# aehogan/lammps-induced-dipole-polarization-pair-style

Measured on AMD Instinct MI355X. Metric: atom-steps/sec, higher is better.
Workload: dtype f64

## Files before the change

lammps-induced-dipole-polarization-pair-style_amd/csrc/lab/api_env_knobs.inc:

```
  if (const char *e = getenv("POLAR_ABLATE")) h->ablate = atoi(e);
  if (const char *e = getenv("POLAR_HOST_COLORS")) h->host_colors = atoi(e) != 0;
  if (const char *e = getenv("POLAR_SWEEP_KERNEL")) h->sweep_kernel = atoi(e);
  if (const char *e = getenv("POLAR_TILE_WAVES")) h->tile_waves = atoi(e) == 8 ? 8 : 4;
  if (const char *e = getenv("POLAR_TILE_WIDE")) h->tile_wide = atoi(e) != 0;
  if (const char *e = getenv("POLAR_CACHE_R2")) h->cache_r2 = atoi(e);
  if (const char *e = getenv("POLAR_LJ_TYPED")) h->lj_typed = atoi(e) != 0;
  if (const char *e = getenv("POLAR_STATIC_XQ")) h->static_xq = atoi(e) != 0;
  if (const char *e = getenv("POLAR_POL_FIRST")) h->pol_first = atoi(e) != 0;
  if (const char *e = getenv("POLAR_LP_WG_PER_CU")) h->lp_wg_per_cu = atoi(e);
  if (const char *e = getenv("POLAR_LP_QM")) h->lp_quad_major = atoi(e) != 0;
  if (const char *e = getenv("POLAR_LP_TILES")) h->lp_tiles = atoi(e) == 1 ? 1 : 2;
  if (const char *e = getenv("POLAR_LP_ROWS")) h->lp_rows = std::max(1, std::min(64, atoi(e)));
  if (const char *e = getenv("POLAR_LP_PAIRS")) h->lp_pairs = atoi(e) != 0;
  if (const char *e = getenv("POLAR_CLUSTER_DIST")) h->cluster_dist = atof(e);
  if (const char *e = getenv("POLAR_CLUSTER_MAX")) h->cluster_max = std::max(1, std::min(4, atoi(e)));
  if (const char *e = getenv("POLAR_LP_DEPTH")) { int v = atoi(e); h->lp_depth = (v == 2 || v == 3) ? v : 0; }
  if (const char *e = getenv("POLAR_QUAD_BLOCK")) { int v = atoi(e); if (v >= 64 && v <= 1024 && v % 64 == 0) h->quad_block = v; }
  if (const char *e = getenv("POLAR_FIELD_BLOCK")) { int v = atoi(e); if (v >= 64 && v <= 1024 && v % 64 == 0) h->field_block = v; }
  if (const char *e = getenv("POLAR_FORCE_LITERAL")) h->force_literal = atoi(e) != 0;
```

lammps-induced-dipole-polarization-pair-style_amd/csrc/polar_handle.hpp:

```cpp
#pragma once
#include <hip/hip_runtime.h>

#include <algorithm>
#include <initializer_list>
#include <utility>
#include <chrono>
#include <cmath>
#include <cstdio>
#include <cstdlib>
#include <exception>
#include <cstring>
#include <numeric>
#include <string>
#include <thread>
#include <mutex>
#include <condition_variable>
#include <functional>
#include <memory>
#include <stdexcept>
#include <unistd.h>
#include <vector>

#include "pair_host.hpp"
#include "polar_kernels.hpp"
// ... 117 lines not shown
  DBuf<double2> d_dd_s;
  DBuf<int2> d_lpdesc;
  DBuf<double> d_lp_pend;
  DBuf<double> d_lp_part;
  int lp_npart = 0;
  DBuf<int> d_slot;
  std::vector<int> h_cl;
  DBuf<int> d_cl_orig, d_cl_cnt, d_cl_wrap, d_cl_tw;
  DBuf<int4> d_cl_s;
  long long cl_pitch = 0;
  int ncl = 0;
  double cluster_dist = 2.0;
  int cluster_max = 4;
  long long cl_slots = 0;
  DBuf<double4> d_xq, d_pos4, d_xq_s;
  long long nl_pairs = 0, dd_pairs = 0;
  long long nl_pitch = 0, dd_pitch = 0;
  DBuf<int> d_overflow;
  DBuf<unsigned long long> d_ddtot;
  int *h_flags = nullptr;
  unsigned long long *h_ddtot = nullptr;
  int inum = 0;
  long long nneigh = 0;
  bool mu_resident = false;
  DBuf<double> d_dbgf;
  DBuf<double> d_acc_x, d_acc_f, d_acc_g, d_acc_dF, d_acc_dG, d_acc_part;
  DBuf<AccelState> d_acc_state;
  long long acc_pitch = 0; int acc_rows = 0;
  DBuf<double> d_mu0;
  bool mu0_saved = false;
  int attempt = 0;
  int last_sweeps = 0;
  bool mu_host_in_sync = false;
  std::vector<int> color_off;
  std::vector<int> color_sub;
  int color_nsub = 1;
  DBuf<int> d_bflag; int bflag_n = 0;
  std::vector<int *> h_nl_stage; std::vector<hipEvent_t> ev_nl;
  hipStream_t up_stream = nullptr; hipEvent_t ev_list_up = nullptr; bool list_up_pending = false;
  std::vector<long long> h_first; std::vector<int> h_nn, h_ilist;
  bool colors_global = false;
  std::vector<int> user_colors;
  bool user_colors_clashed = false;
  std::vector<int> h_rows;
  bool colors_valid = false;
  double color_keep = 2.0;
  bool slots_by_color = false;
  long long color_epoch = 0;
  long long slots_epoch = -1;
  bool colors_recheck = false;
  std::vector<int> h_color;
  DBuf<int> d_color_orig, d_color_s;
  DBuf<int> d_klist;
  DBuf<int> d_cadj, d_cdeg, d_ccnt, d_cflags, d_crelabel;
  DBuf<unsigned long long> d_cprio;
  DBuf<double> d_cstat;
  DBuf<long long> d_coff;
  int *h_cflags = nullptr;
  double *h_cstat = nullptr;
  long long *h_coff = nullptr;
  int cadj_pitch = 16;
  int host_colors = 0;
  int colors_reused = 0, colors_rebuilt = 0;
  double ms_color_host = 0.0;
  double color_dist = 2.4;
  int field_block = 256;
  double bbox_lo[3] = {0, 0, 0}, bbox_hi[3] = {0, 0, 0};
  long long global_count = 0;
  DBuf<double> d_xchg; DBuf<int> d_xidx;
  bool device_list = false;
  int user_full_list = 0;
  long long lj_pitch = 0;
  DBuf<double4> d_ljpos; DBuf<int2> d_ljaux; DBuf<int> d_tag, d_nspecial, d_special, d_ljcell_id, d_ljcell_cnt, d_ljcell_fill; DBuf<long long> d_ljcell_first; DBuf<double> d_cutneighsq;
  int lj_typed = 1;
  bool lj_tab_arith = false;
  int lj_pers = 1;
  int ncu = 0;
  int lj_pers_threads = 768;
  bool sym_typed = false, dev_typed = false;
  int static_xq = 1;
  int pol_first = 1;
#ifdef POLAR_LAB
  int force_literal = 0;
#endif
  int part_k = 0, part_n = 1;
  int lp_wg_per_cu = 0;
  int lp_quad_major = 1;
  int quad_block = POLAR_BLOCK;
  int lp_tiles = 2;
  int lp_rows = 1;
  int lp_pairs = 0;
  DBuf<int> d_ulead, d_udd_j;
  DBuf<long long> d_upos;
  DBuf<int2> d_unit;
  DBuf<int4> d_udesc;
  std::vector<int> unit_off;
  long long upitch = 0;
  int lp_depth = 0;
  int cache_r2 = -1;
  int stream_mode = 1;
  int sweep_kernel = 2;
  int ablate = 0;
  DBuf<SRec> d_srec0, d_srec1;
  DBuf<TileHdr> d_thdr;
  DBuf<TileRowEnt> d_trow;
  DBuf<int> d_un_j;
  DBuf<unsigned short> d_dd16;
  DBuf<double> d_pend;
  int un_pitch = 0;
  int un_lds = 0;
  long long pitch16 = 0;
  int tile_max_u = 0;
  bool tile_reported = false;
  double dens = 0.0;
  std::vector<TileLaunch> tile_launches;
  TileLaunch tile_all{};
  size_t tile_lds_attr[16] = {0, 0, 0, 0, 0, 0, 0, 0, 0, 0, 0, 0, 0, 0, 0, 0};
  size_t tile_build_lds_attr = 0;
  int tile_waves = 4;
  int tile_wide = 0;
  int tile_sw[3] = {2, 2, 2};
  int deterministic = 0;
  Scal *h_scal = nullptr;
  hipEvent_t ev[8] = {};
  hipStream_t lj_stream = nullptr;
  hipEvent_t ev_fork = nullptr, ev_join = nullptr, ev_lj0 = nullptr, ev_lj1 = nullptr, ev_dl0 = nullptr, ev_dl1 = nullptr;
  hipStream_t dl_stream = nullptr;
  hipEvent_t ev_mu_ready = nullptr;
  double *early_mu = nullptr, *early_ef = nullptr, *user_mu = nullptr, *user_ef = nullptr;
  hipEvent_t ev_fchunk[4] = {nullptr, nullptr, nullptr, nullptr};
  bool overlap_lj = true;
  bool lj_forked = false;
  std::vector<double> h_tmp;
  double *h_stage = nullptr;
  DBuf<double> d_trace;
  DBuf<double4> d_ew_kv; DBuf<int4> d_ew_hkl, d_ew_rows;
  DBuf<double2> d_ew_s, d_ew_m, d_ew_part;
  DBuf<double> d_ew_erec, d_ew_vpart, d_ew_out;
  std::vector<double> ew_key;
  int ew_nk = 0, ew_nrow = 0, ew_nm = 0;
  double ew_cell[6] = {0, 0, 0, 0, 0, 0};
  hipEvent_t ev_ks[4] = {nullptr, nullptr, nullptr, nullptr};
  int ntrace = 0;
  size_t h_stage_cap = 0;
};
inline int fail(polar_handle *h, int code, const std::string &m) {
  if (h) h->err = m;
  return code;
}

template <typename F>
int guarded(polar_handle *h, F &&fn) {
  if (!h) return POLAR_ERR_STATE;
  try {
    return fn();
  } catch (const InputError &e) {
    return fail(h, POLAR_ERR_INPUT, e.what());
  } catch (const Unsupported &e) {
    return fail(h, POLAR_ERR_UNSUPPORTED, e.what());
  } catch (const NoDevice &e) {
    return fail(h, POLAR_ERR_NO_DEVICE, e.what());
  } catch (const HipError &e) {
    return fail(h, POLAR_ERR_HIP, e.what());
  } catch (const std::exception &e) {
    return fail(h, POLAR_ERR_STATE, e.what());
  }
// ... 167 lines not shown
```

lammps-induced-dipole-polarization-pair-style_amd/csrc/polar_lists.hpp:

```cpp
#pragma once

#include "polar_common.hpp"

namespace polar {

struct CellGrid {
  int trim;
  int nc[3];
  double lo[3], inv[3];
};

__device__ __forceinline__ int cell_of(const CellGrid &g, const Box &b, double x, double y, double z) {
  int c[3];
  double fr3[3];
  frac_coords(b, g.lo, x, y, z, fr3);
#pragma unroll
  for (int k = 0; k < 3; k++) {
    double fr = fr3[k];
    fr -= floor(fr);
    int ck = (int)(fr * g.nc[k]);
    c[k] = ck >= g.nc[k] ? g.nc[k] - 1 : ck;
  }
  return (c[2] * g.nc[1] + c[1]) * g.nc[0] + c[0];
}
// ... 363 lines not shown
  for (int step = 0; step < budget && k >= 0 && k < m; step++) {
    const unsigned long long ek = __shfl(in, k, 64) & ((1ull << k) - 1ull);
    const bool nb = (ek >> lane) & 1ull;
    unsigned long long ok = __shfl(allow, k, 64);
    for (int c = 0; c < top; c++)
      if (((ok >> c) & 1ull) && __ballot(nb && mycol == c)) ok &= ~(1ull << c);
    const int cur = __shfl(mycol, k, 64);
    if (cur >= 0) ok &= ~((2ull << cur) - 1ull);
    if (ok) {
      const int c = __ffsll((long long)ok) - 1;
      if (lane == k) mycol = c;
      k++;
      if (lane == k) mycol = -1;
    } else {
      if (lane == k) mycol = -1;
      k--;
    }
  }
  if (k >= m && lane < m) color_s[ball[lane]] = mycol;
}
static __global__ void k_color_regroup(int n, const int *__restrict__ deg, const int *__restrict__ class_rank, const int *__restrict__ perm,
                                int *__restrict__ color_s, unsigned long long *__restrict__ prio) {
  const int i = blockIdx.x * blockDim.x + threadIdx.x;
  if (i >= n || deg[i] < 0) return;
  const unsigned o = (unsigned)perm[i];
  prio[i] = ((unsigned long long)(63 - class_rank[color_s[i]]) << 56) | ((unsigned long long)(color_hash(o) >> 8) << 32) | o;
  color_s[i] = -1;
}
static __global__ __launch_bounds__(256) void k_color_stats(int n, const int *__restrict__ color_s, const double *__restrict__ rank,
                                                     double *__restrict__ sums, const int *__restrict__ perm, int own_lo, int own_hi) {
  __shared__ double part[128];
  if (threadIdx.x < 128) part[threadIdx.x] = 0.0;
  __syncthreads();
  const int i = blockIdx.x * blockDim.x + threadIdx.x;
  int c = i < n ? color_s[i] : -1;
  if (c >= 0) { const int o = perm[i]; if (o < own_lo || o >= own_hi) c = -1; }
  if (c >= 0) {
    atomicAdd(&part[2 * c], 1.0);
    atomicAdd(&part[2 * c + 1], rank ? rank[i] : 1.0);
  }
  __syncthreads();
  if (threadIdx.x < 128 && part[threadIdx.x] != 0.0) atomicAdd(sums + threadIdx.x, part[threadIdx.x]);
}
static __global__ void k_color_relabel(int n, const int *__restrict__ relabel, const int *__restrict__ perm, int *__restrict__ color_s,
                                int *__restrict__ color_orig) {
  const int i = blockIdx.x * blockDim.x + threadIdx.x;
  if (i >= n) return;
  const int c = color_s[i] >= 0 ? relabel[color_s[i]] : -1;
  color_s[i] = c;
  color_orig[perm[i]] = c;
}
__device__ __forceinline__ int color_class(int j, const int *__restrict__ color_s, const int *__restrict__ perm, int own_lo, int own_hi,
                                           const int *__restrict__ sub, int nsub) {
  const int c = color_s[j];
  if (c < 0) return -1;
  const int o = perm[j];
  if (o < own_lo || o >= own_hi) return -1;
  return sub ? nsub * c + sub[o] : c;
}
static __global__ void k_color_cellcount(long long ncell, int nclass, const long long *__restrict__ cell_first, const int *__restrict__ npol,
                                  const int *__restrict__ color_s, int *__restrict__ cnt, const int *__restrict__ perm, int own_lo, int own_hi,
                                  const int *__restrict__ sub, int nsub) {
  const long long c = blockIdx.x * (long long)blockDim.x + threadIdx.x;
  if (c >= ncell) return;
  const int a = (int)cell_first[c], e = a + npol[c];
  for (int q = 0; q < nclass; q++) {
    int k = 0;
    for (int j = a; j < e; j++) k += color_class(j, color_s, perm, own_lo, own_hi, sub, nsub) == q;
    cnt[(size_t)q * ncell + c] = k;
  }
}
static __global__ void k_color_fill(long long ncell, int nclass, const long long *__restrict__ cell_first, const int *__restrict__ npol,
                             const int *__restrict__ color_s, const int *__restrict__ perm, const long long *__restrict__ off,
                             int *__restrict__ rows_orig, int own_lo, int own_hi, const int *__restrict__ sub, int nsub) {
  const long long c = blockIdx.x * (long long)blockDim.x + threadIdx.x;
  if (c >= ncell) return;
  const int a = (int)cell_first[c], e = a + npol[c];
  for (int q = 0; q < nclass; q++) {
    long long w = off[(size_t)q * ncell + c];
    for (int j = a; j < e; j++) if (color_class(j, color_s, perm, own_lo, own_hi, sub, nsub) == q) rows_orig[w++] = perm[j];
  }
}

template <bool TRI, bool RECHECK>
static __global__ __launch_bounds__(POLAR_BLOCK) void k_nl_build(const int *__restrict__ rows, int nrows,
                                                          const double4 *__restrict__ pos4, Box box, CellGrid g,
                                                          const long long *__restrict__ cell_first, double cutallsq,
                                                          double ddcutsq, long long nl_pitch, long long dd_pitch,
                                                          int *__restrict__ nl_cnt, int *__restrict__ dd_cnt,
                                                          int *__restrict__ nl_j, int *__restrict__ dd_j,
                                                          double *__restrict__ dd_r2, int pad_dd,
                                                          int dd_shift_qm, int dd_pad_index, int *__restrict__ dd_wrap,
                                                          const int *__restrict__ color_s, double colordistsq,
                                                          int *__restrict__ color_conflict,
                                                          const int *__restrict__ dd_slot,
                                                          int *__restrict__ overflow,
                                                          unsigned long long *__restrict__ dd_total) {
  const int dd_shift = dd_shift_qm & 255, dd_qm = dd_shift_qm >> 8;
  const int lane = threadIdx.x & 63;
  const int row = blockIdx.x * POLAR_ROWS_PER_BLOCK + (threadIdx.x >> 6);
  if (row >= nrows) return;
  const int i = rows ? rows[row] : row;
  const double4 ri = pos4[i];
  const int imol = __double2hiint(ri.w), ipol = __double2loint(ri.w);
  const int icol = (RECHECK && color_s && ipol) ? color_s[i] : -2;
  bool clash = RECHECK && color_s && ipol && icol < 0;
  int cc[3];
  double uu[3], edge[3];
  {
    double fr3[3];
    frac_coords(box, g.lo, ri.x, ri.y, ri.z, fr3);
#pragma unroll
    for (int k = 0; k < 3; k++) {
      double fr = fr3[k];
      fr -= floor(fr);
      const double t = fr * g.nc[k];
      int ck = (int)t;
      ck = ck >= g.nc[k] ? g.nc[k] - 1 : ck;
      cc[k] = __builtin_amdgcn_readfirstlane(ck);
      uu[k] = wave_uniform(t - ck); edge[k] = wave_uniform(box.prd[k] / g.nc[k]);
    }
  }
  const int c0 = cc[0], c1 = cc[1], c2 = cc[2];
  const int slot_i = dd_slot ? dd_slot[i] : i;
  const long long nl0 = (long long)i * nl_pitch, dd0 = (long long)(slot_i >= 0 ? slot_i : 0) * dd_pitch;
  int ncount = 0, dcount = 0;
  bool wrap_lane = false;
  const unsigned long long below = (lane == 0) ? 0ull : (~0ull >> (64 - lane));
  const int n0 = g.nc[0], n1 = g.nc[1], n2 = g.nc[2];
  const int zlo = n2 >= 5 ? c2 - 2 : 0, zcnt = n2 >= 5 ? 5 : n2;
  const int ylo = n1 >= 5 ? c1 - 2 : 0, ycnt = n1 >= 5 ? 5 : n1;
  const double reach = sqrt(cutallsq > ddcutsq ? cutallsq : ddcutsq) + 1e-6;
  const double reach2 = wave_uniform(reach * reach);
  const int nsr = zcnt * ycnt;
  int ra0 = 0, rb0 = 0, ra1 = 0, rb1 = 0;
  if (lane < nsr) {
    const int zz = zlo + lane / ycnt, yy = ylo + lane % ycnt;
    int b2 = zz, b1 = yy;
    bool ok = true;
    if (b2 < 0 || b2 >= n2) { if (!box.periodic[2]) ok = false; b2 = (b2 + n2) % n2; }
    if (b1 < 0 || b1 >= n1) { if (!box.periodic[1]) ok = false; b1 = (b1 + n1) % n1; }
    double dzmin = 0.0, dymin = 0.0;
    if (n2 >= 5) { const int d = zz - c2; dzmin = d > 0 ? (d - uu[2]) * edge[2] : (d < 0 ? (uu[2] - (d + 1)) * edge[2] : 0.0); }
    if (n1 >= 5) { const int d = yy - c1; dymin = d > 0 ? (d - uu[1]) * edge[1] : (d < 0 ? (uu[1] - (d + 1)) * edge[1] : 0.0); }
    const double rem2 = reach2 - dzmin * dzmin - dymin * dymin;
    if (g.trim && rem2 < 0.0) ok = false;
    int xlo = n0 >= 5 ? c0 - 2 : 0, xhi = n0 >= 5 ? c0 + 2 : n0 - 1;
    if (ok && g.trim && n0 >= 5) {
      const double xr = sqrt(rem2) / edge[0];
      int lo_off = (int)floor(uu[0] - xr), hi_off = (int)floor(uu[0] + xr);
      lo_off = lo_off < -2 ? -2 : lo_off; hi_off = hi_off > 2 ? 2 : hi_off;
      xlo = c0 + lo_off; xhi = c0 + hi_off;
    }
    if (ok) {
      const long long rowbase = ((long long)b2 * n1 + b1) * n0;
      const int xa = xlo < 0 ? 0 : xlo, xb = xhi >= n0 ? n0 - 1 : xhi;
      ra0 = (int)cell_first[rowbase + xa]; rb0 = (int)cell_first[rowbase + xb + 1];
      if (box.periodic[0]) {
        if (xlo < 0) { ra1 = (int)cell_first[rowbase + xlo + n0]; rb1 = (int)cell_first[rowbase + n0]; }
        else if (xhi >= n0) { ra1 = (int)cell_first[rowbase]; rb1 = (int)cell_first[rowbase + xhi - n0 + 1]; }
      }
    }
  }
  for (int sr = 0; sr < nsr; sr++) {
#pragma unroll
    for (int piece = 0; piece < 2; piece++) {
      const int a = __builtin_amdgcn_readlane(piece ? ra1 : ra0, sr), b = __builtin_amdgcn_readlane(piece ? rb1 : rb0, sr);
      for (int base = a; base < b; base += 64) {
        const int p = base + lane;
        bool in_nl = false, in_dd = false;
        const int j = p;
        int same = 0;
        double rsq = 0.0;
        if (p < b && j != i) {
          const double4 rj = pos4[j];
          double ex, ey, ez;
          const bool shifted = min_image_rint_w<TRI>(box, ri.x, ri.y, ri.z, rj.x, rj.y, rj.z, ex, ey, ez);
          rsq = ex * ex + ey * ey + ez * ez;
          in_nl = rsq <= cutallsq;
          in_dd = ipol && slot_i >= 0 && __double2loint(rj.w) && (rsq < ddcutsq);
          if (RECHECK && icol >= 0 && rsq < colordistsq && __double2loint(rj.w) && color_s[j] == icol) clash = true;
          wrap_lane |= in_dd && shifted;
          same = (imol != 0 && imol == __double2hiint(rj.w)) ? POLAR_NL_SAMEMOL : 0;
        }
        const unsigned long long m_nl = __ballot(in_nl), m_dd = __ballot(in_dd);
        const int kn = ncount + __popcll(m_nl & below), kd = dcount + __popcll(m_dd & below);
        if (in_nl && kn < nl_pitch) nl_j[nl0 + kn] = j | same;
        if (in_dd && kd < dd_pitch) {
          dd_j[dd0 + (dd_shift ? lp_slot(kd, dd_qm) : (long long)kd)] = j << dd_shift;
          if (dd_r2) dd_r2[dd0 + kd] = rsq;
        }
        ncount += __popcll(m_nl);
        dcount += __popcll(m_dd);
      }
    }
  }
  if (pad_dd) {
    const int have = dcount < dd_pitch ? dcount : (int)dd_pitch;
    const int padded = (have + 63) & ~63;
    for (int k = have + lane; k < padded; k += 64) {
      dd_j[dd0 + (dd_shift ? lp_slot(k, dd_qm) : (long long)k)] = (dd_pad_index >= 0 ? dd_pad_index : i) << dd_shift;
      if (dd_r2) dd_r2[dd0 + k] = 1e60;
    }
  }
  if (RECHECK && color_s && __ballot(clash) != 0ull && lane == 0) atomicOr(color_conflict, 1);
  const unsigned long long anywrap = __ballot(wrap_lane);
  if (lane == 0) {
    nl_cnt[i] = ncount; dd_cnt[i] = dcount;
    if (dd_wrap) dd_wrap[i] = anywrap != 0ull;
    if (ncount > nl_pitch || dcount > dd_pitch) atomicMax(overflow, ncount > dcount ? ncount : dcount);
    if (dcount) atomicAdd(dd_total + (blockIdx.x & 63) * 16, (unsigned long long)(dcount < dd_pitch ? dcount : (int)dd_pitch));
  }
}

#ifdef POLAR_LAB
#include "lab/lists_paired_rows.hpp"
#endif

#ifdef POLAR_LAB
#include "lab/lists_cluster_rows.hpp"
#endif

struct LJGrid {
  int nc[3];
  double lo[3], inv[3];
};
__device__ __forceinline__ int lj_cell_of(const LJGrid &g, double x, double y, double z) {
  const double p[3] = {x, y, z};
  int c[3];
#pragma unroll
  for (int k = 0; k < 3; k++) {
    int ck = (int)floor((p[k] - g.lo[k]) * g.inv[k]);
    c[k] = ck < 0 ? 0 : (ck >= g.nc[k] ? g.nc[k] - 1 : ck);
  }
  return (c[2] * g.nc[1] + c[1]) * g.nc[0] + c[0];
}
static __global__ void k_lj_cell_count(int nall, const double *__restrict__ x, LJGrid g, int *__restrict__ cell_id,
                                int *__restrict__ cell_cnt) {
  int i = blockIdx.x * blockDim.x + threadIdx.x;
  if (i >= nall) return;
  const int c = lj_cell_of(g, x[3 * i], x[3 * i + 1], x[3 * i + 2]);
  cell_id[i] = c;
  atomicAdd(&cell_cnt[c], 1);
}
static __global__ void k_lj_cell_fill(int nall, const int *__restrict__ cell_id, const long long *__restrict__ cell_first,
                               int *__restrict__ fill, const double *__restrict__ x, const int *__restrict__ type,
                               const int *__restrict__ mol, const int *__restrict__ tag, double4 *__restrict__ pos,
                               int2 *__restrict__ aux) {
  int i = blockIdx.x * blockDim.x + threadIdx.x;
  if (i >= nall) return;
  const int c = cell_id[i];
  const int s = (int)cell_first[c] + atomicAdd(&fill[c], 1);
  pos[s] = make_double4(x[3 * i], x[3 * i + 1], x[3 * i + 2], __hiloint2double(mol[i], type[i]));
  aux[s] = make_int2(i, tag ? tag[i] : i + 1);
}

static __global__ __launch_bounds__(POLAR_BLOCK) void k_lj_nl_build(int row_lo, int nrows, int ntypes, const double *__restrict__ x,
                                                             const int *__restrict__ type, const int *__restrict__ mol,
                                                             const double4 *__restrict__ pos, const int2 *__restrict__ aux,
                                                             LJGrid g, const long long *__restrict__ cell_first,
                                                             const double *__restrict__ cutneighsq, Box box,
                                                             int exclude_intra, const int *__restrict__ nspecial,
                                                             const int *__restrict__ special, int maxspecial, int sf1,
                                                             int sf2, int sf3, long long pitch, int *__restrict__ cnt,
                                                             int *__restrict__ out_j, int *__restrict__ overflow,
                                                             unsigned long long *__restrict__ total, int typed) {
  extern __shared__ double cn_lds[];
  const int w = ntypes + 1;
  for (int t = threadIdx.x; t < w * w; t += blockDim.x) cn_lds[t] = cutneighsq[t];
  __syncthreads();
  const int lane = threadIdx.x & 63;
  const int r_ = blockIdx.x * POLAR_ROWS_PER_BLOCK + (threadIdx.x >> 6);
  if (r_ >= nrows) return;
  const int i = row_lo + r_;
  const double xi = x[3 * i], yi = x[3 * i + 1], zi = x[3 * i + 2];
  const int itype = type[i], imol = mol[i];
  const double *cn = cn_lds + itype * w;
  int n1 = 0, n2 = 0, n3 = 0;
  if (nspecial) { n1 = nspecial[3 * i]; n2 = nspecial[3 * i + 1]; n3 = nspecial[3 * i + 2]; }
  const int *sp = special ? special + (size_t)i * maxspecial : nullptr;
  const int ci = lj_cell_of(g, xi, yi, zi);
  const int n0 = g.nc[0], n1c = g.nc[1], n2c = g.nc[2];
  const int c0 = ci % n0, c1 = (ci / n0) % n1c, c2 = ci / (n0 * n1c);
  const unsigned long long below = (lane == 0) ? 0ull : (~0ull >> (64 - lane));
  const long long row0 = (long long)i * pitch;
  int count = 0;
  for (int zz = max(c2 - 2, 0); zz <= min(c2 + 2, n2c - 1); zz++)
    for (int yy = max(c1 - 2, 0); yy <= min(c1 + 2, n1c - 1); yy++) {
      const long long rb = ((long long)zz * n1c + yy) * n0;
      const long long a = cell_first[rb + max(c0 - 2, 0)], b = cell_first[rb + min(c0 + 2, n0 - 1) + 1];
      for (long long base = a; base < b; base += 64) {
        const long long p = base + lane;
        bool keep = false;
        int entry = 0;
        if (p < b) {
          const double4 pj = pos[p];
// ... 166 lines not shown
```

lammps-induced-dipole-polarization-pair-style_amd/csrc/polar_step.hip:

```cpp
#include "polar_handle.hpp"

void launch_scan(long long n, const int *in, long long *out, DBuf<long long> &tot, hipStream_t s) {
  const int nb = (int)std::max<long long>(1, (n + POLAR_SCAN_ITEMS - 1) / POLAR_SCAN_ITEMS);
  tot.ensure((size_t)nb + 1);
  k_scan_block<<<nb, 1024, 0, s>>>(n, in, out, tot.p);
  if (nb > 1) {
    k_scan_totals<<<1, 1024, 0, s>>>(nb, tot.p, out + n);
    k_scan_add<<<nblk(n - POLAR_SCAN_ITEMS, 256), 256, 0, s>>>(n, out, tot.p);
  }
}

void build_cells(polar_handle *h) {
  const polar_settings &st = h->ph.st;
  const int n = h->nlocal;
  const double cutall = std::max(st.cut_coul, st.dd_cutoff);
  double width[3];
  box_widths(h->box, width);
  for (int k = 0; k < 3; k++)
    if (h->box.periodic[k] && width[k] < 2.0 * cutall * (1.0 - 1e-12))
      throw InputError("dd_cutoff mode needs box lengths >= 2*max(cut_coul,dd_cutoff); use exact mode (dd_cutoff 0)");
  CellGrid &g = h->grid;
  g.trim = 1;
#ifdef POLAR_LAB
  if (const char *e = getenv("POLAR_NL_TRIM")) g.trim = atoi(e);
// ... 56 lines not shown
  h->d_slot.ensure(n + 1);
  HIPCHECK(hipMemsetAsync(h->d_slot.p, 0xFF, (size_t)(n + 1) * sizeof(int), s));
  if (gs && h->colors_valid) {
    const int tot = h->color_off.empty() ? 0 : h->color_off.back();
    if (tot > 0) k_slot_from_rows<<<nblk(tot, 256), 256, 0, s>>>(tot, h->d_rows.p, h->d_slot.p);
    h->slots_by_color = true;
    h->slots_epoch = h->color_epoch;
  } else {
    k_slot_from_rows<<<nblk(own_n(h), 256), 256, 0, s>>>(own_n(h), own_rows(h), h->d_slot.p);
    h->slots_by_color = false;
  }
}

void build_lists(polar_handle *h) {
  const polar_settings &st = h->ph.st;
  const int n = h->nlocal;
  const double cutall = std::max(st.cut_coul, st.dd_cutoff);
  hipStream_t s = h->stream;
  const CellGrid &g = h->grid;
  if (h->nl_pitch == 0 && getenv("POLAR_INIT_PITCH")) h->nl_pitch = h->dd_pitch = ((std::max(64, atoi(getenv("POLAR_INIT_PITCH"))) + 63) / 64) * 64;
  if (h->nl_pitch == 0) {
    double vol = h->box.prd[0] * h->box.prd[1] * h->box.prd[2];
    {
      int nc[3];
      long long tot = 1;
      for (int k = 0; k < 3; k++) { nc[k] = std::max(1, std::min(64, (int)(h->box.prd[k] / cutall))); tot *= nc[k]; }
      std::vector<char> occ((size_t)tot, 0);
      for (int a = 0; a < n; a++) {
        long long c = 0, mul = 1;
        for (int k = 0; k < 3; k++) {
          double fr = (h->hx[3 * (size_t)a + k] - h->grid.lo[k]) / h->box.prd[k];
          fr -= std::floor(fr);
          c += mul * std::min(nc[k] - 1, (int)(fr * nc[k]));
          mul *= nc[k];
        }
        occ[(size_t)c] = 1;
      }
      long long filled = 0;
      for (char v : occ) filled += v;
      if (filled > 0) vol *= (double)filled / (double)tot;
    }
    h->dens = n / vol;
    double mean = n / vol * 4.18879020478639 * cutall * cutall * cutall;
    h->nl_pitch = h->dd_pitch = (((long long)(1.5 * mean) + 64) / 64 + 1) * 64;
  }
  if (h->sweep_kernel == 2) h->dd_pitch = ((h->dd_pitch + 255) / 256) * 256;
  if ((h->sweep_kernel == 2 || h->sweep_kernel == 3) && ((long long)n + 1) * (long long)sizeof(AtomRec) >= (1ll << 31))
    throw InputError("more than 2^25 atoms on one handle: the 32-bit record offsets of the sweep's index stream would wrap (shard the system)");
  h->d_nl_cnt.ensure(n + 1); h->d_dd_cnt.ensure(n + 1);
  h->d_nl_j.ensure((size_t)n * h->nl_pitch + 64);
  if (h->sweep_kernel < 3) h->d_dd_j.ensure((size_t)n * h->dd_pitch + 1024);
  else h->d_dd_j.ensure(64);
  int mode = h->cache_r2;
  if (h->sweep_kernel == 1) mode = 0;
  if (h->sweep_kernel == 2) mode = 3;
  if (h->sweep_kernel >= 3) mode = 4;
  if (mode < 0) {
    const double est_pairs = h->dd_pairs > 0 ? (double)h->dd_pairs : 0.35 * (double)own_n(h) * (double)h->dd_pitch;
    mode = (12.0 * est_pairs < 200.0e6) ? 1 : 2;
  }
  h->stream_mode = mode;
  const bool r2c = mode == 1;
  if (mode == 1) h->d_dd_r2.ensure((size_t)n * h->dd_pitch + 64);
  else if (mode == 0) h->d_dd_s.ensure((size_t)n * h->dd_pitch + 64);
  double *r2p = r2c ? h->d_dd_r2.p : nullptr;
  double2 *sp = mode == 0 ? h->d_dd_s.p : nullptr;
  bool fuse = mode != 0 && mode != 4;
#ifdef POLAR_LAB
  if (getenv("POLAR_NO_FUSE_R2")) fuse = false;
#endif
  const double cutallsq = cutall * cutall, ddsq = mode == 4 ? -1.0 : st.dd_cutoff * st.dd_cutoff;
  const int nr = own_n(h);
  const int *rows = own_rows(h);
  zero_many(s, {{h->d_nl_cnt.p, (size_t)(n + 1) * sizeof(int)}, {h->d_dd_cnt.p, (size_t)(n + 1) * sizeof(int)},
                {h->d_overflow.p, 16 * sizeof(int)}, {h->d_ddtot.p, 64 * 16 * sizeof(unsigned long long)}});
  const bool lp = mode == 3;
  if (lp) h->d_dd_wrap.ensure(n + 1);
  const bool recheck = h->colors_valid && h->colors_recheck && h->sweep_kernel < 3 && (int)h->h_color.size() == n;
  if (h->colors_recheck && !recheck) { h->colors_valid = false; h->colors_recheck = false; }
  if (recheck) {
    h->d_color_s.ensure(n + 1);
    k_color_map<<<nblk(n, 256), 256, 0, s>>>(n, h->d_perm.p, h->d_color_orig.p, h->d_color_s.p);
  }
#define NLB(TRI, RC)                                                                                                          \
  k_nl_build<TRI, RC><<<nblk(nr, POLAR_ROWS_PER_BLOCK), POLAR_BLOCK, 0, s>>>(                                                 \
      rows, nr, h->d_pos4.p, h->box, g, h->d_cell_first.p, cutallsq, ddsq, h->nl_pitch, h->dd_pitch, h->d_nl_cnt.p,            \
      h->d_dd_cnt.p, h->d_nl_j.p, h->d_dd_j.p, fuse ? r2p : nullptr, fuse ? 1 : 0, lp ? (6 | (h->lp_quad_major << 8)) : 0,    \
      lp ? n : -1, lp ? h->d_dd_wrap.p : nullptr, recheck ? h->d_color_s.p : nullptr, h->color_keep * h->color_keep,           \
      h->d_overflow.p + 8, lp ? h->d_slot.p : nullptr, h->d_overflow.p, h->d_ddtot.p)
  if (h->box.triclinic) { if (recheck) NLB(true, true); else NLB(true, false); }
  else                  { if (recheck) NLB(false, true); else NLB(false, false); }
#undef NLB
  const RowList ddl{h->d_dd_cnt.p, h->dd_pitch};
  if (fuse || mode == 4) {
  }
#ifdef POLAR_LAB
  else if (st.damping_type == POLAR_DAMP_EXPONENTIAL)
    k_dd_scalars<0><<<nblk(nr, POLAR_ROWS_PER_BLOCK), POLAR_BLOCK, 0, s>>>(rows, nr, h->d_rec0.p, h->box, ddl, h->d_dd_j.p, st.polar_damp, sp, r2p);
  else
    k_dd_scalars<1><<<nblk(nr, POLAR_ROWS_PER_BLOCK), POLAR_BLOCK, 0, s>>>(rows, nr, h->d_rec0.p, h->box, ddl, h->d_dd_j.p, st.polar_damp, sp, r2p);
#endif
  HIPCHECK(hipMemcpyAsync(h->h_flags, h->d_overflow.p, sizeof(int), hipMemcpyDeviceToHost, s));
  HIPCHECK(hipMemcpyAsync(h->h_ddtot, h->d_ddtot.p, 64 * 16 * sizeof(unsigned long long), hipMemcpyDeviceToHost, s));
}
template <bool AP>
static void launch_rank(polar_handle *h, int pass) {
  const int n = h->nlocal, ntot = h->nlocal + h->nghost;
  dim3 grid(nblk(n, POLAR_ROWS_PER_BLOCK)), block(POLAR_BLOCK);
  if (pass == 2) k_fold_scal<<<1, POLAR_NSLOT, 0, h->stream>>>(h->d_scal.p, h->d_slots.p, 1);
  const int nchunk = (AP && pass == 1) ? std::max(1, std::min(16, 8192 / std::max(n, 1))) : 1;
  if (pass == 1)
    k_rank<AP, 1><<<nblk((long long)n * nchunk, POLAR_ROWS_PER_BLOCK), block, 0, h->stream>>>(n, ntot, h->d_x.p, h->d_alpha.p, h->d_mol.p, h->box, RowList{h->d_nl_cnt.p, h->nl_pitch},
                                                 h->d_nl_j.p, h->d_rec0.p, h->d_mol_s.p, h->d_scal.p, h->d_slots.p, h->d_rank.p, nchunk);
  else
    k_rank<AP, 2><<<grid, block, 0, h->stream>>>(n, ntot, h->d_x.p, h->d_alpha.p, h->d_mol.p, h->box, RowList{h->d_nl_cnt.p, h->nl_pitch},
                                                 h->d_nl_j.p, h->d_rec0.p, h->d_mol_s.p, h->d_scal.p, h->d_slots.p, h->d_rank.p, 1);
}

void launch_rank_pass(polar_handle *h, bool allpairs, int pass) {
  if (allpairs) launch_rank<true>(h, pass); else launch_rank<false>(h, pass);
}

template <bool AP, int DAMP, int EP>
void launch_field(polar_handle *h, int nrows, const int *rows) {
  const polar_settings &st = h->ph.st;
  if (nrows <= 0) return;
  const int fb = h->field_block;
  const size_t lds = AP ? 0 : (size_t)(fb / 64) * 64 * 5 * sizeof(double2);
  k_field<AP, DAMP, EP><<<nblk(nrows, fb / 64), fb, lds, h->stream>>>(
      nrows, rows, h->nlocal, h->d_rec0.p, h->d_rec1.p, h->box, RowList{h->d_dd_cnt.p, h->dd_pitch}, h->d_dd_j.p, h->d_dd_s.p,
      st.dd_cutoff * st.dd_cutoff, st.polar_damp, h->d_ef_s.p, h->d_F.p, h->d_scal.p, h->d_slots.p
#ifdef POLAR_LAB
      , h->ablate
#endif
      );
}
template <int EP>
void launch_field_dyn(polar_handle *h, bool ap, int nrows, const int *rows) {
  const bool expd = h->ph.st.damping_type == POLAR_DAMP_EXPONENTIAL;
  if (ap) { if (expd) launch_field<true, 0, EP>(h, nrows, rows); else launch_field<true, 1, EP>(h, nrows, rows); }
#ifdef POLAR_LAB
  else    { if (expd) launch_field<false, 0, EP>(h, nrows, rows); else launch_field<false, 1, EP>(h, nrows, rows); }
#else
  else throw std::logic_error("k_field's list branch exists in the lab build only");
#endif
}

#ifdef POLAR_LAB
#include "lab/launch_quad.inc"
#else
template <int EP> inline void launch_field_quad(polar_handle *, int, const int *) { throw std::logic_error("lab build only"); }
#endif

void prepare_lp(polar_handle *h) {
  const polar_settings &st = h->ph.st;
  const bool gs = st.polar_gs || st.polar_gs_ranked;
  const int tot = gs ? (h->color_off.empty() ? 0 : h->color_off.back()) : own_n(h);
  h->d_lpdesc.ensure((size_t)tot + 1);
  h->lp_npart = 0;
  if (deterministic(h)) {
    h->d_lp_pend.ensure(4 * (size_t)tot + 4);
    const int nlaunch = gs ? (int)h->color_off.size() - 1 : 1;
    h->lp_npart = tot / 256 + nlaunch + 1;
    h->d_lp_part.ensure((size_t)h->lp_npart + 1);
    HIPCHECK(hipMemsetAsync(h->d_lp_part.p, 0, (size_t)h->lp_npart * sizeof(double), h->stream));
  }
  if (tot > 0)
    k_lp_desc<<<nblk(tot, 256), 256, 0, h->stream>>>(tot, gs ? h->d_rows.p : own_rows(h), RowList{h->d_dd_cnt.p, h->dd_pitch},
                                                     h->d_dd_wrap.p, h->d_lpdesc.p);
}
template <int EP>
void launch_field_lp(polar_handle *h, int nrows, const int2 *desc) {
  const long long row0 = desc - h->d_lpdesc.p;
  if (nrows <= 0) return;
  const polar_settings &st = h->ph.st;
// ... 810 lines not shown
```

Baseline: 16.23 million.

## Compact cell-row runs and stage neighbor-list writes through LDS queues

```diff
diff --git a/lammps-induced-dipole-polarization-pair-style_amd/csrc/lab/api_env_knobs.inc b/lammps-induced-dipole-polarization-pair-style_amd/csrc/lab/api_env_knobs.inc
--- a/lammps-induced-dipole-polarization-pair-style_amd/csrc/lab/api_env_knobs.inc
+++ b/lammps-induced-dipole-polarization-pair-style_amd/csrc/lab/api_env_knobs.inc
@@ -18,3 +18,4 @@
   if (const char *e = getenv("POLAR_QUAD_BLOCK")) { int v = atoi(e); if (v >= 64 && v <= 1024 && v % 64 == 0) h->quad_block = v; }
   if (const char *e = getenv("POLAR_FIELD_BLOCK")) { int v = atoi(e); if (v >= 64 && v <= 1024 && v % 64 == 0) h->field_block = v; }
   if (const char *e = getenv("POLAR_FORCE_LITERAL")) h->force_literal = atoi(e) != 0;
+  if (const char *e = getenv("POLAR_NL_PARENT")) h->nl_parent = atoi(e) != 0;
diff --git a/lammps-induced-dipole-polarization-pair-style_amd/csrc/lab/lists_nl_build_parent.hpp b/lammps-induced-dipole-polarization-pair-style_amd/csrc/lab/lists_nl_build_parent.hpp
--- /dev/null
+++ b/lammps-induced-dipole-polarization-pair-style_amd/csrc/lab/lists_nl_build_parent.hpp
@@ -0,0 +1,130 @@
+template <bool TRI, bool RECHECK>
+static __global__ __launch_bounds__(POLAR_BLOCK) void k_nl_build_parent(const int *__restrict__ rows, int nrows,
+                                                          const double4 *__restrict__ pos4, Box box, CellGrid g,
+                                                          const long long *__restrict__ cell_first, double cutallsq,
+                                                          double ddcutsq, long long nl_pitch, long long dd_pitch,
+                                                          int *__restrict__ nl_cnt, int *__restrict__ dd_cnt,
+                                                          int *__restrict__ nl_j, int *__restrict__ dd_j,
+                                                          double *__restrict__ dd_r2, int pad_dd,
+                                                          int dd_shift_qm, int dd_pad_index, int *__restrict__ dd_wrap,
+                                                          const int *__restrict__ color_s, double colordistsq,
+                                                          int *__restrict__ color_conflict,
+                                                          const int *__restrict__ dd_slot,
+                                                          int *__restrict__ overflow,
+                                                          unsigned long long *__restrict__ dd_total) {
+  const int dd_shift = dd_shift_qm & 255, dd_qm = dd_shift_qm >> 8;
+  const int lane = threadIdx.x & 63;
+  const int row = blockIdx.x * POLAR_ROWS_PER_BLOCK + (threadIdx.x >> 6);
+  if (row >= nrows) return;
+  const int i = rows ? rows[row] : row;
+  const double4 ri = pos4[i];
+  const int imol = __double2hiint(ri.w), ipol = __double2loint(ri.w);
+  const int icol = (RECHECK && color_s && ipol) ? color_s[i] : -2;
+  bool clash = RECHECK && color_s && ipol && icol < 0;
+  int cc[3];
+  double uu[3], edge[3];
+  {
+    double fr3[3];
+    frac_coords(box, g.lo, ri.x, ri.y, ri.z, fr3);
+#pragma unroll
+    for (int k = 0; k < 3; k++) {
+      double fr = fr3[k];
+      fr -= floor(fr);
+      const double t = fr * g.nc[k];
+      int ck = (int)t;
+      ck = ck >= g.nc[k] ? g.nc[k] - 1 : ck;
+      cc[k] = __builtin_amdgcn_readfirstlane(ck);
+      uu[k] = wave_uniform(t - ck); edge[k] = wave_uniform(box.prd[k] / g.nc[k]);
+    }
+  }
+  const int c0 = cc[0], c1 = cc[1], c2 = cc[2];
+  const int slot_i = dd_slot ? dd_slot[i] : i;
+  const long long nl0 = (long long)i * nl_pitch, dd0 = (long long)(slot_i >= 0 ? slot_i : 0) * dd_pitch;
+  int ncount = 0, dcount = 0;
+  bool wrap_lane = false;
+  const unsigned long long below = (lane == 0) ? 0ull : (~0ull >> (64 - lane));
+  const int n0 = g.nc[0], n1 = g.nc[1], n2 = g.nc[2];
+  const int zlo = n2 >= 5 ? c2 - 2 : 0, zcnt = n2 >= 5 ? 5 : n2;
+  const int ylo = n1 >= 5 ? c1 - 2 : 0, ycnt = n1 >= 5 ? 5 : n1;
+  const double reach = sqrt(cutallsq > ddcutsq ? cutallsq : ddcutsq) + 1e-6;
+  const double reach2 = wave_uniform(reach * reach);
+  const int nsr = zcnt * ycnt;
+  int ra0 = 0, rb0 = 0, ra1 = 0, rb1 = 0;
+  if (lane < nsr) {
+    const int zz = zlo + lane / ycnt, yy = ylo + lane % ycnt;
+    int b2 = zz, b1 = yy;
+    bool ok = true;
+    if (b2 < 0 || b2 >= n2) { if (!box.periodic[2]) ok = false; b2 = (b2 + n2) % n2; }
+    if (b1 < 0 || b1 >= n1) { if (!box.periodic[1]) ok = false; b1 = (b1 + n1) % n1; }
+    double dzmin = 0.0, dymin = 0.0;
+    if (n2 >= 5) { const int d = zz - c2; dzmin = d > 0 ? (d - uu[2]) * edge[2] : (d < 0 ? (uu[2] - (d + 1)) * edge[2] : 0.0); }
+    if (n1 >= 5) { const int d = yy - c1; dymin = d > 0 ? (d - uu[1]) * edge[1] : (d < 0 ? (uu[1] - (d + 1)) * edge[1] : 0.0); }
+    const double rem2 = reach2 - dzmin * dzmin - dymin * dymin;
+    if (g.trim && rem2 < 0.0) ok = false;
+    int xlo = n0 >= 5 ? c0 - 2 : 0, xhi = n0 >= 5 ? c0 + 2 : n0 - 1;
+    if (ok && g.trim && n0 >= 5) {
+      const double xr = sqrt(rem2) / edge[0];
+      int lo_off = (int)floor(uu[0] - xr), hi_off = (int)floor(uu[0] + xr);
+      lo_off = lo_off < -2 ? -2 : lo_off; hi_off = hi_off > 2 ? 2 : hi_off;
+      xlo = c0 + lo_off; xhi = c0 + hi_off;
+    }
+    if (ok) {
+      const long long rowbase = ((long long)b2 * n1 + b1) * n0;
+      const int xa = xlo < 0 ? 0 : xlo, xb = xhi >= n0 ? n0 - 1 : xhi;
+      ra0 = (int)cell_first[rowbase + xa]; rb0 = (int)cell_first[rowbase + xb + 1];
+      if (box.periodic[0]) {
+        if (xlo < 0) { ra1 = (int)cell_first[rowbase + xlo + n0]; rb1 = (int)cell_first[rowbase + n0]; }
+        else if (xhi >= n0) { ra1 = (int)cell_first[rowbase]; rb1 = (int)cell_first[rowbase + xhi - n0 + 1]; }
+      }
+    }
+  }
+  for (int sr = 0; sr < nsr; sr++) {
+#pragma unroll
+    for (int piece = 0; piece < 2; piece++) {
+      const int a = __builtin_amdgcn_readlane(piece ? ra1 : ra0, sr), b = __builtin_amdgcn_readlane(piece ? rb1 : rb0, sr);
+      for (int base = a; base < b; base += 64) {
+        const int p = base + lane;
+        bool in_nl = false, in_dd = false;
+        const int j = p;
+        int same = 0;
+        double rsq = 0.0;
+        if (p < b && j != i) {
+          const double4 rj = pos4[j];
+          double ex, ey, ez;
+          const bool shifted = min_image_rint_w<TRI>(box, ri.x, ri.y, ri.z, rj.x, rj.y, rj.z, ex, ey, ez);
+          rsq = ex * ex + ey * ey + ez * ez;
+          in_nl = rsq <= cutallsq;
+          in_dd = ipol && slot_i >= 0 && __double2loint(rj.w) && (rsq < ddcutsq);
+          if (RECHECK && icol >= 0 && rsq < colordistsq && __double2loint(rj.w) && color_s[j] == icol) clash = true;
+          wrap_lane |= in_dd && shifted;
+          same = (imol != 0 && imol == __double2hiint(rj.w)) ? POLAR_NL_SAMEMOL : 0;
+        }
+        const unsigned long long m_nl = __ballot(in_nl), m_dd = __ballot(in_dd);
+        const int kn = ncount + __popcll(m_nl & below), kd = dcount + __popcll(m_dd & below);
+        if (in_nl && kn < nl_pitch) nl_j[nl0 + kn] = j | same;
+        if (in_dd && kd < dd_pitch) {
+          dd_j[dd0 + (dd_shift ? lp_slot(kd, dd_qm) : (long long)kd)] = j << dd_shift;
+          if (dd_r2) dd_r2[dd0 + kd] = rsq;
+        }
+        ncount += __popcll(m_nl);
+        dcount += __popcll(m_dd);
+      }
+    }
+  }
+  if (pad_dd) {
+    const int have = dcount < dd_pitch ? dcount : (int)dd_pitch;
+    const int padded = (have + 63) & ~63;
+    for (int k = have + lane; k < padded; k += 64) {
+      dd_j[dd0 + (dd_shift ? lp_slot(k, dd_qm) : (long long)k)] = (dd_pad_index >= 0 ? dd_pad_index : i) << dd_shift;
+      if (dd_r2) dd_r2[dd0 + k] = 1e60;
+    }
+  }
+  if (RECHECK && color_s && __ballot(clash) != 0ull && lane == 0) atomicOr(color_conflict, 1);
+  const unsigned long long anywrap = __ballot(wrap_lane);
+  if (lane == 0) {
+    nl_cnt[i] = ncount; dd_cnt[i] = dcount;
+    if (dd_wrap) dd_wrap[i] = anywrap != 0ull;
+    if (ncount > nl_pitch || dcount > dd_pitch) atomicMax(overflow, ncount > dcount ? ncount : dcount);
+    if (dcount) atomicAdd(dd_total + (blockIdx.x & 63) * 16, (unsigned long long)(dcount < dd_pitch ? dcount : (int)dd_pitch));
+  }
+}
diff --git a/lammps-induced-dipole-polarization-pair-style_amd/csrc/polar_handle.hpp b/lammps-induced-dipole-polarization-pair-style_amd/csrc/polar_handle.hpp
--- a/lammps-induced-dipole-polarization-pair-style_amd/csrc/polar_handle.hpp
+++ b/lammps-induced-dipole-polarization-pair-style_amd/csrc/polar_handle.hpp
@@ -223,6 +223,7 @@
   int pol_first = 1;
 #ifdef POLAR_LAB
   int force_literal = 0;
+  int nl_parent = 0;
 #endif
   int part_k = 0, part_n = 1;
   int lp_wg_per_cu = 0;
diff --git a/lammps-induced-dipole-polarization-pair-style_amd/csrc/polar_lists.hpp b/lammps-induced-dipole-polarization-pair-style_amd/csrc/polar_lists.hpp
--- a/lammps-induced-dipole-polarization-pair-style_amd/csrc/polar_lists.hpp
+++ b/lammps-induced-dipole-polarization-pair-style_amd/csrc/polar_lists.hpp
@@ -469,7 +469,8 @@
   }
 }
 
-template <bool TRI, bool RECHECK>
+#define POLAR_NLQ 128
+template <bool TRI, bool RECHECK, bool R2>
 static __global__ __launch_bounds__(POLAR_BLOCK) void k_nl_build(const int *__restrict__ rows, int nrows,
                                                           const double4 *__restrict__ pos4, Box box, CellGrid g,
                                                           const long long *__restrict__ cell_first, double cutallsq,
@@ -483,11 +484,14 @@
                                                           const int *__restrict__ dd_slot,
                                                           int *__restrict__ overflow,
                                                           unsigned long long *__restrict__ dd_total) {
+  __shared__ unsigned s_queue[POLAR_ROWS_PER_BLOCK][2][POLAR_NLQ];
   const int dd_shift = dd_shift_qm & 255, dd_qm = dd_shift_qm >> 8;
   const int lane = threadIdx.x & 63;
-  const int row = blockIdx.x * POLAR_ROWS_PER_BLOCK + (threadIdx.x >> 6);
+  const int wv = __builtin_amdgcn_readfirstlane(threadIdx.x >> 6);
+  const int row = blockIdx.x * POLAR_ROWS_PER_BLOCK + wv;
   if (row >= nrows) return;
-  const int i = rows ? rows[row] : row;
+  unsigned *const qn = s_queue[wv][0], *const qd = s_queue[wv][1];
+  const int i = __builtin_amdgcn_readfirstlane(rows ? rows[row] : row);
   const double4 ri = pos4[i];
   const int imol = __double2hiint(ri.w), ipol = __double2loint(ri.w);
   const int icol = (RECHECK && color_s && ipol) ? color_s[i] : -2;
@@ -511,8 +515,6 @@
   const int c0 = cc[0], c1 = cc[1], c2 = cc[2];
   const int slot_i = dd_slot ? dd_slot[i] : i;
   const long long nl0 = (long long)i * nl_pitch, dd0 = (long long)(slot_i >= 0 ? slot_i : 0) * dd_pitch;
-  int ncount = 0, dcount = 0;
-  bool wrap_lane = false;
   const unsigned long long below = (lane == 0) ? 0ull : (~0ull >> (64 - lane));
   const int n0 = g.nc[0], n1 = g.nc[1], n2 = g.nc[2];
   const int zlo = n2 >= 5 ? c2 - 2 : 0, zcnt = n2 >= 5 ? 5 : n2;
@@ -549,49 +551,112 @@
       }
     }
   }
-  for (int sr = 0; sr < nsr; sr++) {
-#pragma unroll
-    for (int piece = 0; piece < 2; piece++) {
-      const int a = __builtin_amdgcn_readlane(piece ? ra1 : ra0, sr), b = __builtin_amdgcn_readlane(piece ? rb1 : rb0, sr);
-      for (int base = a; base < b; base += 64) {
-        const int p = base + lane;
-        bool in_nl = false, in_dd = false;
-        const int j = p;
-        int same = 0;
-        double rsq = 0.0;
-        if (p < b && j != i) {
-          const double4 rj = pos4[j];
-          double ex, ey, ez;
-          const bool shifted = min_image_rint_w<TRI>(box, ri.x, ri.y, ri.z, rj.x, rj.y, rj.z, ex, ey, ez);
-          rsq = ex * ex + ey * ey + ez * ez;
-          in_nl = rsq <= cutallsq;
-          in_dd = ipol && slot_i >= 0 && __double2loint(rj.w) && (rsq < ddcutsq);
-          if (RECHECK && icol >= 0 && rsq < colordistsq && __double2loint(rj.w) && color_s[j] == icol) clash = true;
-          wrap_lane |= in_dd && shifted;
-          same = (imol != 0 && imol == __double2hiint(rj.w)) ? POLAR_NL_SAMEMOL : 0;
-        }
-        const unsigned long long m_nl = __ballot(in_nl), m_dd = __ballot(in_dd);
-        const int kn = ncount + __popcll(m_nl & below), kd = dcount + __popcll(m_dd & below);
-        if (in_nl && kn < nl_pitch) nl_j[nl0 + kn] = j | same;
-        if (in_dd && kd < dd_pitch) {
-          dd_j[dd0 + (dd_shift ? lp_slot(kd, dd_qm) : (long long)kd)] = j << dd_shift;
-          if (dd_r2) dd_r2[dd0 + kd] = rsq;
-        }
-        ncount += __popcll(m_nl);
-        dcount += __popcll(m_dd);
-      }
-    }
-  }
+  int rdelta, rend, nrun, total;
+  {
+    const int a0 = __shfl(ra0, lane >> 1, 64), l0 = __shfl(rb0 - ra0, lane >> 1, 64);
+    const int a1 = __shfl(ra1, lane >> 1, 64), l1 = __shfl(rb1 - ra1, lane >> 1, 64);
+    int start = (lane & 1) ? a1 : a0, len = (lane & 1) ? l1 : l0;
+    const unsigned long long mrun = __ballot(len > 0);
+    nrun = __popcll(mrun);
+    const int dst = len > 0 ? __popcll(mrun & below) : nrun + __popcll(~mrun & below);
+    start = __builtin_amdgcn_ds_permute(dst << 2, start);
+    len = __builtin_amdgcn_ds_permute(dst << 2, len);
+    rend = len;
+#pragma unroll
+    for (int off = 1; off < 64; off <<= 1) {
+      const int up = __shfl_up(rend, off, 64);
+      if (lane >= off) rend += up;
+    }
+    rdelta = start - (rend - len);
+    total = __builtin_amdgcn_readlane(rend, 63);
+  }
+  const double inv0 = box.periodic[0] ? box.inv[0] : 0.0, inv1 = box.periodic[1] ? box.inv[1] : 0.0,
+               inv2 = box.periodic[2] ? box.inv[2] : 0.0;
+  const double ddcut_i = (ipol && slot_i >= 0) ? ddcutsq : -1.0;
+  const int lslot = (int)(dd_shift ? lp_slot(lane, dd_qm) : (long long)lane);
+  int nq = 0, nfl = 0, dq = 0, dfl = 0;
+  int dr2 = 0;
+  unsigned wacc = 0u;
+  auto flush_dd = [&](const int cnt) {
+    __builtin_amdgcn_fence(__ATOMIC_ACQ_REL, "wavefront");
+    __builtin_amdgcn_wave_barrier();
+    const int k = dfl + lane;
+    const unsigned e = qd[k & (POLAR_NLQ - 1)];
+    int *const out = dd_j + (dd0 + (dd_shift ? lp_slot(dfl, dd_qm) : (long long)dfl));
+    if (lane < cnt && k < dd_pitch) out[lslot] = (int)(e << dd_shift);
+    dfl += 64;
+  };
+  auto flush_nl = [&](const int cnt) {
+    __builtin_amdgcn_fence(__ATOMIC_ACQ_REL, "wavefront");
+    __builtin_amdgcn_wave_barrier();
+    const int k = nfl + lane;
+    const unsigned e = qn[k & (POLAR_NLQ - 1)];
+    int *const out = nl_j + (nl0 + nfl);
+    if (lane < cnt && k < nl_pitch) out[lane] = (int)(e & 0x7FFFFFFFu);
+    const bool d = lane < cnt && (e >> 31);
+    const unsigned long long m_dd = __ballot(d);
+    if (d) qd[(dq + __popcll(m_dd & below)) & (POLAR_NLQ - 1)] = e & POLAR_NL_MASK;
+    dq += __popcll(m_dd);
+    nfl += 64;
+    while (dq - dfl >= 64) flush_dd(64);
+  };
+  int cur = 0;
+  int s_end = __builtin_amdgcn_readlane(rend, 0), s_delta = __builtin_amdgcn_readlane(rdelta, 0);
+  for (int base = 0; base < total; base += 64) {
+    const int q = base + lane;
+    int j = q + s_delta;
+    while (s_end < base + 64 && cur + 1 < nrun) {
+      cur++;
+      s_delta = __builtin_amdgcn_readlane(rdelta, cur);
+      j = q >= s_end ? q + s_delta : j;
+      s_end = __builtin_amdgcn_readlane(rend, cur);
+    }
+    bool in_nl = false, in_dd = false;
+    unsigned e = 0u;
+    double rsq = 0.0;
+    if (q < total && j != i) {
+      const double4 rj = pos4[j];
+      double ex = ri.x - rj.x, ey = ri.y - rj.y, ez = ri.z - rj.z;
+      const double nz = rint(ez * inv2);
+      ez = fma(-box.prd[2], nz, ez);
+      if (TRI) { ey = fma(-box.yz, nz, ey); ex = fma(-box.xz, nz, ex); }
+      const double ny = rint(ey * inv1);
+      ey = fma(-box.prd[1], ny, ey);
+      if (TRI) ex = fma(-box.xy, ny, ex);
+      const double nx = rint(ex * inv0);
+      ex = fma(-box.prd[0], nx, ex);
+      rsq = ex * ex + ey * ey + ez * ez;
+      in_nl = rsq <= cutallsq;
+      const int jpol = __double2loint(rj.w);
+      in_dd = jpol && (rsq < ddcut_i);
+      if (RECHECK && icol >= 0 && rsq < colordistsq && jpol && color_s[j] == icol) clash = true;
+      wacc |= in_dd ? (unsigned)(__double2hiint(nx) | __double2hiint(ny) | __double2hiint(nz)) : 0u;
+      e = (unsigned)j | ((imol != 0 && imol == __double2hiint(rj.w)) ? (unsigned)POLAR_NL_SAMEMOL : 0u) | (in_dd ? 0x80000000u : 0u);
+    }
+    if (R2) {
+      const unsigned long long m_dd = __ballot(in_dd);
+      const int kd = dr2 + __popcll(m_dd & below);
+      if (in_dd && kd < dd_pitch) dd_r2[dd0 + kd] = rsq;
+      dr2 += __popcll(m_dd);
+    }
+    const unsigned long long m_nl = __ballot(in_nl);
+    if (in_nl) qn[(nq + __popcll(m_nl & below)) & (POLAR_NLQ - 1)] = e;
+    nq += __popcll(m_nl);
+    while (nq - nfl >= 64) flush_nl(64);
+  }
+  if (nq > nfl) flush_nl(nq - nfl);
+  if (dq > dfl) flush_dd(dq - dfl);
+  const int ncount = nq, dcount = dq;
   if (pad_dd) {
     const int have = dcount < dd_pitch ? dcount : (int)dd_pitch;
     const int padded = (have + 63) & ~63;
     for (int k = have + lane; k < padded; k += 64) {
       dd_j[dd0 + (dd_shift ? lp_slot(k, dd_qm) : (long long)k)] = (dd_pad_index >= 0 ? dd_pad_index : i) << dd_shift;
-      if (dd_r2) dd_r2[dd0 + k] = 1e60;
+      if (R2) dd_r2[dd0 + k] = 1e60;
     }
   }
   if (RECHECK && color_s && __ballot(clash) != 0ull && lane == 0) atomicOr(color_conflict, 1);
-  const unsigned long long anywrap = __ballot(wrap_lane);
+  const unsigned long long anywrap = __ballot((wacc & 0x7FFFFFFFu) != 0u);
   if (lane == 0) {
     nl_cnt[i] = ncount; dd_cnt[i] = dcount;
     if (dd_wrap) dd_wrap[i] = anywrap != 0ull;
@@ -599,6 +664,10 @@
     if (dcount) atomicAdd(dd_total + (blockIdx.x & 63) * 16, (unsigned long long)(dcount < dd_pitch ? dcount : (int)dd_pitch));
   }
 }
+
+#ifdef POLAR_LAB
+#include "lab/lists_nl_build_parent.hpp"
+#endif
 
 #ifdef POLAR_LAB
 #include "lab/lists_paired_rows.hpp"
diff --git a/lammps-induced-dipole-polarization-pair-style_amd/csrc/polar_step.hip b/lammps-induced-dipole-polarization-pair-style_amd/csrc/polar_step.hip
--- a/lammps-induced-dipole-polarization-pair-style_amd/csrc/polar_step.hip
+++ b/lammps-induced-dipole-polarization-pair-style_amd/csrc/polar_step.hip
@@ -162,15 +162,23 @@
     h->d_color_s.ensure(n + 1);
     k_color_map<<<nblk(n, 256), 256, 0, s>>>(n, h->d_perm.p, h->d_color_orig.p, h->d_color_s.p);
   }
-#define NLB(TRI, RC)                                                                                                          \
-  k_nl_build<TRI, RC><<<nblk(nr, POLAR_ROWS_PER_BLOCK), POLAR_BLOCK, 0, s>>>(                                                 \
+#define NLB_K(...)                                                                                                            \
+  __VA_ARGS__<<<nblk(nr, POLAR_ROWS_PER_BLOCK), POLAR_BLOCK, 0, s>>>(                                                         \
       rows, nr, h->d_pos4.p, h->box, g, h->d_cell_first.p, cutallsq, ddsq, h->nl_pitch, h->dd_pitch, h->d_nl_cnt.p,            \
       h->d_dd_cnt.p, h->d_nl_j.p, h->d_dd_j.p, fuse ? r2p : nullptr, fuse ? 1 : 0, lp ? (6 | (h->lp_quad_major << 8)) : 0,    \
       lp ? n : -1, lp ? h->d_dd_wrap.p : nullptr, recheck ? h->d_color_s.p : nullptr, h->color_keep * h->color_keep,           \
       h->d_overflow.p + 8, lp ? h->d_slot.p : nullptr, h->d_overflow.p, h->d_ddtot.p)
+#define NLB_NEW(TRI, RC) do { if (fuse && r2p) NLB_K(k_nl_build<TRI, RC, true>); else NLB_K(k_nl_build<TRI, RC, false>); } while (0)
+#ifdef POLAR_LAB
+#define NLB(TRI, RC) do { if (h->nl_parent) NLB_K(k_nl_build_parent<TRI, RC>); else NLB_NEW(TRI, RC); } while (0)
+#else
+#define NLB(TRI, RC) NLB_NEW(TRI, RC)
+#endif
   if (h->box.triclinic) { if (recheck) NLB(true, true); else NLB(true, false); }
   else                  { if (recheck) NLB(false, true); else NLB(false, false); }
 #undef NLB
+#undef NLB_NEW
+#undef NLB_K
   const RowList ddl{h->d_dd_cnt.p, h->dd_pitch};
   if (fuse || mode == 4) {
   }
```

Result: no change. 16.40 million, median of 2 (+1.0%).
